# pixeli99/SVD_Xtend

Hardware: AMD Instinct MI355X
Metric: train-step samples/sec (14-frame 512x320 fp16 SVD UNet) (higher is better)
Workload: dtype fp16; 1 GPU; SVD UNet train step, 14 frames 512x320, batch 1/GPU, 1524623082 params (397620480 trainable: temporal_transformer_block*), fwd + EDM loss + bwd + grad all-reduce + AdamW; global_batch=1, grad_accum=1, parallelism=dp1, grad_allreduce=none, ranks_seen=1, allreduce_bytes=1590482176, exec=hipgraph, gemm_tuning_sweeps=0, gemm_variant=4

## Files before the change

include/svdx.h:

```cpp
#ifndef SVDX_H
#define SVDX_H
#include <stddef.h>
#include <stdint.h>

#ifdef __cplusplus
extern "C" {
#endif

#define SVDX_F16 0
#define SVDX_BF16 1

#define SVDX_OUT_ACT 0
#define SVDX_OUT_F32 1
#define SVDX_OUT_F32_ATOMIC 2
#define SVDX_OUT_F32_ADD 4
#define SVDX_OUT_F32_SLAB 3

#define SVDX_EPI_NONE 0
#define SVDX_EPI_GEGLU_FWD 1
#define SVDX_EPI_GEGLU_BWD 2

#define SVDX_GATHER_PLAIN 0
#define SVDX_GATHER_CONV3X3 1
#define SVDX_GATHER_CONV3X3_DGRAD2 2
#define SVDX_GATHER_TEMPORAL3 3
#define SVDX_GATHER_CONV3X3_PAD0 4

typedef struct svdx_gather {
    int mode;
    int n_img;
    int hi, wi;
    int ho, wo;
    int cin;
    int stride;
    int ups;
    int t, hw;
    int lda;
} svdx_gather;

#define SVDX_VERSION 614
int         svdx_version(void);
int         svdx_last_error(char* buf, size_t n);
int         svdx_device_ok(void);

int svdx_gemm(const void* A, const void* B, void* C, int M, int N, int K, int lda, int ldb, int ldc,
              const float* bias, const float* rowvec, int rv_ld, int rv_rows_per_group, int rv_mod,
              const void* res, int ldres, const svdx_gather* gather, const void* zero_page,
              int out_mode, float alpha, int split_k, int variant, int epilogue, const void* aux_in, void* aux_out, int aux_dim,
              int dtype, void* stream);
int svdx_gemm_tile(int variant, int M, int N, int split_k, int epilogue, int aux_dim, int* geom);

int svdx_gemm_gn(const void* A, const void* B, void* C, int M, int N, int K, int lda, int ldb, int ldc,
                 const float* bias, const float* rowvec, int rv_ld, int rv_rows_per_group, int rv_mod,
                 const void* res, int ldres, const svdx_gather* gather, const void* zero_page,
                 float alpha, int variant, float* gn_stats, int gn_rows, int gn_cg, int dtype, void* stream);

int svdx_gemm_dual(const void* A, const void* B, void* C, int M, int N, int K, int lda, int ldb, int ldc,
                   const float* bias, const float* rowvec, int rv_ld, int rv_rows_per_group, int rv_mod,
                   const void* res, int ldres, const svdx_gather* gather, const void* zero_page,
                   int out_mode, float alpha, int variant, const void* A2, const void* B2, int K2, int lda2, int ldb2,
                   int a2_seg_n, int dtype, void* stream);

#define SVDX_TN_FLAT 64
int svdx_gemm_tn(const void* A, const void* B, float* C, int R, int N, int K, int lda, int ldb, int ldc,
                 float* a_colsum, const void* zero_page, int out_mode, int split_k, int stages, float* found_inf, int dtype, void* stream);

int svdx_gemm_tn_gather(const void* A, const void* X, float* C, int R, int N, int lda, int ldc, const svdx_gather* gather,
                        float* a_colsum, int out_mode, int split_k, int stages, float* found_inf, int dtype, void* stream);

int svdx_conv_wgrad_finalize(const float* acc, int nsplit, int64_t slab_stride, int ld_acc, float* w_grad, int cout, int cin, int cin_p,
                             int taps, float alpha, int store, const float* colsum_slabs, int colsum_ld, float* b_grad, float* found_inf,
                             void* stream);

// ... 85 lines not shown
                     const float* lse, const float* D, void* dq, int nb, int heads, int S,
                     int ld, int ld_o, int ld_d, float scale, int dtype, void* stream);

int svdx_tattn_fwd(const void* q, const void* k, const void* v, void* o, int B, int T, int HW, int heads,
                   int ld, int ld_o, float scale, int dtype, void* stream);
int svdx_tattn_bwd(const void* q, const void* k, const void* v, const void* d_o, void* dq, void* dk, void* dv,
                   int B, int T, int HW, int heads, int ld, int ld_o, int ld_d, float scale, int dtype, void* stream);

int svdx_geglu_fwd(const void* pre, void* out, int M, int F, int dtype, void* stream);
int svdx_geglu_bwd(const void* dout, const void* pre, void* dpre, int M, int F, int dtype, void* stream);
int svdx_add(const void* a, const void* b, void* out, int64_t n, int dtype, void* stream);
int svdx_blend(const void* a, const void* b, const float* mix_factor, void* out, int64_t n, int dtype, void* stream);
int svdx_blend_bwd(const void* dy, const float* mix_factor, void* da, void* db, int64_t n, int dtype, void* stream);
int svdx_add_rowvec(const void* x, const float* vec, void* out, int rows, int C, int rv_ld,
                    int rows_per_group, int mod, int dtype, void* stream);
#define SVDX_COLSUM_SLAB 512
int svdx_colsum(const void* x, float* out, int rows, int C, int ldx, int n_groups, int rows_per_group, int mod,
                int accumulate, float* scratch, int dtype, void* stream);
int svdx_transpose(const void* in, int ld_in, void* out, int ld_out, int rows, int cols, int dtype, void* stream);
int svdx_concat2(const void* a, int Ca, const void* b, int Cb, void* out, int rows, int dtype, void* stream);
int svdx_split2(const void* in, void* a, int Ca, void* b, int Cb, int rows, int dtype, void* stream);
int svdx_sum2x2(const void* in, void* out, int n_img, int h, int w, int C, int dtype, void* stream);
int svdx_cast_from_f32(const float* in, void* out, int64_t n, int dtype, void* stream);
int svdx_cast_transpose_from_f32(const float* in, void* out, int R, int Ccols, int dtype, void* stream);
int svdx_nchw_to_rows(const float* in, void* out, int n_img, int C, int H, int W, int ld, float mul, int dtype, void* stream);
int svdx_rows_to_nchw(const void* in, float* out, int n_img, int C, int H, int W, int ld, int dtype, void* stream);
int svdx_zero(void* p, size_t bytes, void* stream);

int svdx_tsa_pixels_per_band(int T, int HW);
int svdx_tsa_fwd(const void* x, const float* gamma, const float* beta, float eps, const void* wqkv, const void* wo, const float* bo,
                 const float* cvec, int rv_ld, int rv_rows_per_group, int rv_mod, void* n1, float* stats, void* qkv, void* o, void* h1,
                 int B, int T, int HW, int C, int heads, float scale, int dtype, void* stream);

int svdx_patch_rows(const float* in, void* out, int n_img, int C, int H, int W, int kh, int kw, int stride, int pad, int ho, int wo,
                    int ldk, float mul, int dtype, void* stream);
int svdx_softmax_rows(const void* in, void* out, int rows, int cols, int cols_out, int64_t ld_in, int64_t ld_out, float scale,
                      int dtype, void* stream);
int svdx_act_rows(const void* in, void* out, int64_t n, int act, int dtype, void* stream);
int svdx_blur_axis(const float* in, float* out, int planes, int H, int W, const float* taps, int ntaps, int axis, void* stream);
int svdx_bicubic_affine(const float* in, float* out, int n_img, int C, int H, int W, int ho, int wo, const float* scale,
                        const float* shift, void* stream);
int svdx_attn_small_fwd(const void* qkv, void* out, int n_img, int S, int heads, int d, int dp, int64_t ld, int64_t ld_o, float scale,
                        int dtype, void* stream);
int svdx_zero_spans(float* base, const int* spans, int n_spans, void* stream);
int svdx_stamp(uint64_t* slot, void* stream);
int svdx_wall_clock_khz(void);

int     svdx_plan_begin(void);
int     svdx_plan_end(void** plan);
int64_t svdx_plan_launches(const void* plan);
int64_t svdx_plan_bytes(const void* plan);
int     svdx_plan_replay(const void* plan, void* stream);
int     svdx_plan_free(void* plan);

#define SVDX_MAX_PEERS 16
int svdx_allreduce_grads(float* const* peers, int world, int rank, int64_t n, int phase, void* stream);

#define SVDX_EDM_LOSS_SCRATCH 1024
int svdx_edm_loss(const void* pred, int ld, const float* noisy, const float* target, const float* sigma,
                  float* loss, void* dpred, int B, int T, int C, int HW, const float* opt_state, float* scratch,
                  int dtype, void* stream);

#define SVDX_OPT_STATE_FLOATS 16
#define SVDX_SCHED_CONSTANT 0
#define SVDX_SCHED_CONSTANT_WITH_WARMUP 1
#define SVDX_SCHED_LINEAR 2
// ... 35 lines not shown
```

svd_xtend_amd/build.py:

```python
from __future__ import annotations

import os
import subprocess
import sys
from concurrent.futures import ThreadPoolExecutor

HERE = os.path.dirname(os.path.abspath(__file__))
CSRC = os.path.join(HERE, "csrc")
SOURCES = ["common.cpp", "gemm_nt.hip", "gemm_tn.hip", "gemm_small.hip", "norm.hip", "elementwise.hip", "attention.hip", "tattn.hip", "optim.hip", "encoders.hip", "tsa.hip", "latent.hip", "conv_wgrad.hip"]
FLAGS = ["--offload-arch=gfx950", "-O3", "-std=c++17", "-fPIC", "-Wno-unused-value"]
LIB = os.path.join(CSRC, "libsvdx.so")


def _stale(out: str, deps) -> bool:
    if not os.path.exists(out):
        return True
    t = os.path.getmtime(out)
    return any(os.path.getmtime(d) > t for d in deps)


def build(force: bool = False, verbose: bool = False) -> str:
    hipcc = os.environ.get("HIPCC", "/opt/rocm/bin/hipcc")
    hdrs = sorted(os.path.join(CSRC, f) for f in os.listdir(CSRC) if f.endswith(".h")) + [os.path.join(HERE, "..", "include", "svdx.h")]
    objs = []

    def compile_one(src):
        s = os.path.join(CSRC, src)
        o = os.path.join(CSRC, os.path.splitext(src)[0] + ".o")
        if force or _stale(o, [s] + hdrs):
            cmd = [hipcc] + FLAGS + (["-x", "hip"] if src.endswith(".cpp") else []) + ["-c", s, "-o", o]
            if verbose:
                print(" ".join(cmd), flush=True)
            r = subprocess.run(cmd, capture_output=True, text=True)
            if r.returncode != 0:
                raise RuntimeError(f"hipcc failed on {src}:\n{r.stderr}")
        return o

    with ThreadPoolExecutor(max_workers=6) as ex:
        objs = list(ex.map(compile_one, SOURCES))
    if force or _stale(LIB, objs):
        cmd = [hipcc, "--offload-arch=gfx950", "-shared", "-fPIC", "-o", LIB] + objs
        r = subprocess.run(cmd, capture_output=True, text=True)
# ... 8 lines not shown
```

svd_xtend_amd/kernels.py:

```python
from __future__ import annotations

import ctypes
import os
from dataclasses import dataclass
from typing import Optional

import torch

_HERE = os.path.dirname(os.path.abspath(__file__))
LIB_PATH = os.environ.get("SVDX_LIB") or os.path.join(_HERE, "csrc", "libsvdx.so")

F16, BF16 = 0, 1
OUT_ACT, OUT_F32, OUT_F32_ATOMIC, OUT_F32_SLAB, OUT_F32_ADD = 0, 1, 2, 3, 4
EPI_NONE, EPI_GEGLU_FWD, EPI_GEGLU_BWD = 0, 1, 2
LN_PARTIAL_ROWS = 2048
GN_REPLICAS = 8
GN_STAT_FLOATS = 4
GATHER_PLAIN, GATHER_CONV3X3, GATHER_CONV3X3_DGRAD2, GATHER_TEMPORAL3, GATHER_CONV3X3_PAD0 = 0, 1, 2, 3, 4
ABI_VERSION = 614
OPT_STATE_FLOATS = 16
SCHED_KINDS = {"constant": 0, "constant_with_warmup": 1, "linear": 2, "cosine": 3, "cosine_with_restarts": 4, "polynomial": 5, "piecewise_constant": 6}
SCHED_MAX_RULES = 8
OPT_STATE_ALLOC = 40


class SvdxError(RuntimeError):
    pass


class _LinJobC(ctypes.Structure):
    _fields_ = [("X", ctypes.c_void_p), ("W", ctypes.c_void_p), ("bias", ctypes.c_void_p), ("Y", ctypes.c_void_p),
                ("N", ctypes.c_int), ("K", ctypes.c_int), ("ldw", ctypes.c_int), ("flags", ctypes.c_int)]


class _OuterJobC(ctypes.Structure):
    _fields_ = [("dY", ctypes.c_void_p), ("X", ctypes.c_void_p), ("dW", ctypes.c_void_p),
                ("N", ctypes.c_int), ("K", ctypes.c_int), ("scale", ctypes.c_float), ("reserved", ctypes.c_int)]


class _GradFinJobC(ctypes.Structure):
    _fields_ = [("acc", ctypes.c_void_p), ("dst", ctypes.c_void_p), ("colsum_slabs", ctypes.c_void_p), ("colsum_out", ctypes.c_void_p),
                ("slab_stride", ctypes.c_int64), ("count", ctypes.c_int64), ("nsplit", ctypes.c_int), ("colsum_n", ctypes.c_int),
                ("store", ctypes.c_int), ("reserved", ctypes.c_int), ("found_inf", ctypes.c_void_p)]


class _LnRedJobC(ctypes.Structure):
    _fields_ = [("partial", ctypes.c_void_p), ("dgamma", ctypes.c_void_p), ("dbeta", ctypes.c_void_p),
                ("nblk", ctypes.c_int), ("C", ctypes.c_int)]


class _GatherC(ctypes.Structure):
    _fields_ = [(n, ctypes.c_int) for n in
# ... 21 lines not shown


_SIGS = {
    "svdx_gemm": "ppp" "iiiiii" "p" "piii" "pi" "pp" "ifii" "ippi" "ip",
    "svdx_gemm_dual": "ppp" "iiiiii" "p" "piii" "pi" "pp" "ifi" "pp" "iiii" "ip",
    "svdx_gemm_gn": "ppp" "iiiiii" "p" "piii" "pi" "pp" "fi" "pii" "ip",
    "svdx_gemm_tn": "ppp" "iiiiii" "pp" "iii" "p" "ip",
    "svdx_gemm_tn_gather": "ppp" "iiii" "pp" "iii" "p" "ip",
    "svdx_conv_wgrad_finalize": "pil" "ip" "iiii" "fi" "pi" "pp" "p",
    "svdx_conv_pack": "pf" "pp" "iiiii" "i" "pp" "ip",
    "svdx_gemm_finalize": "pil" "pi" "iii" "pp" "iii" "pi" "ppi" "ip",
    "svdx_gemm_finalize_gn": "pil" "p" "iii" "pp" "iii" "pi" "pii" "ip",
    "svdx_small_linear": "pppp" "iiii" "iii" "ip",
    "svdx_outer_acc": "ppp" "iii" "f" "p",
    "svdx_small_linear_batch": "p" "iii" "ip",
    "svdx_outer_acc_batch": "p" "ii" "p",
    "svdx_ln_param_reduce_batch": "p" "i" "p",
    "svdx_grad_finalize_batch": "p" "i" "p",
    "svdx_timestep_embed": "pp" "ii" "p",
    "svdx_gn_stats": "pp" "iiii" "i" "ip",
    "svdx_gn_apply": "ppppp" "iiii" "fi" "ip",
    "svdx_gn_bwd_stats": "pppppp" "iiii" "fi" "i" "ip",
    "svdx_gn_bwd_apply": "pppppppp" "iiii" "fi" "ip",
    "svdx_gn_bwd_stats_affine": "ppppppppp" "iiii" "fi" "ii" "ip",
    "svdx_ln_fwd": "ppppp" "ii" "f" "ip",
    "svdx_ln_bwd": "pppppp" "f" "pppp" "iii" "ip",
    "svdx_attn_fwd": "ppppp" "iiiii" "f" "ip",
    "svdx_attn_bwd_prep": "ppp" "iii" "i" "ip",
    "svdx_attn_bwd_dkv": "pppppppp" "iiiiii" "f" "ip",
    "svdx_attn_bwd_dq": "ppppppp" "iiiiii" "f" "ip",
    "svdx_tattn_fwd": "pppp" "iiii" "ii" "f" "ip",
    "svdx_tattn_bwd": "ppppppp" "iiii" "iii" "f" "ip",
    "svdx_tsa_fwd": "ppp" "f" "ppp" "piii" "ppppp" "iiiii" "f" "ip",
    "svdx_geglu_fwd": "pp" "ii" "ip",
    "svdx_geglu_bwd": "ppp" "ii" "ip",
    "svdx_add": "ppp" "l" "ip",
    "svdx_blend": "pppp" "l" "ip",
    "svdx_blend_bwd": "pppp" "l" "ip",
    "svdx_add_rowvec": "ppp" "iiiii" "ip",
    "svdx_colsum": "pp" "iiiiiii" "p" "ip",
    "svdx_transpose": "pi" "pi" "ii" "ip",
    "svdx_concat2": "pi" "pi" "p" "i" "ip",
    "svdx_split2": "p" "pi" "pi" "i" "ip",
    "svdx_sum2x2": "pp" "iiii" "ip",
    "svdx_cast_from_f32": "pp" "l" "ip",
    "svdx_cast_transpose_from_f32": "pp" "ii" "ip",
    "svdx_nchw_to_rows": "pp" "iiiii" "f" "ip",
    "svdx_rows_to_nchw": "pp" "iiiii" "ip",
    "svdx_zero": "pzp",
    "svdx_patch_rows": "pp" "iiiiiiiiii" "i" "f" "ip",
    "svdx_softmax_rows": "pp" "iii" "ll" "f" "ip",
    "svdx_act_rows": "pp" "l" "i" "ip",
    "svdx_blur_axis": "pp" "iii" "p" "ii" "p",
    "svdx_bicubic_affine": "pp" "iiiiii" "pp" "p",
    "svdx_attn_small_fwd": "pp" "iiiii" "ll" "f" "ip",
    "svdx_stamp": "pp",
    "svdx_zero_spans": "pp" "ip",
    "svdx_edm_loss": "pi" "ppppp" "iiii" "pp" "ip",
    "svdx_check_finite": "plpp",
    "svdx_check_finite_spans": "pp" "i" "pp",
    "svdx_optim_prep": "p" "ffff" "ii" "p",
    "svdx_adamw": "pppp" "l" "dddddd" "pp" "iip",
    "svdx_adamw_tiled": "ppppp" "i" "dddddd" "ppp" "iip",
    "svdx_ema_lerp": "pp" "l" "f" "p",
    "svdx_latent_batch": "pp" "i" "p" "pp" "pp" "ppp" "f" "ppp" "iii" "p",
    "svdx_grad_sumsq_spans": "pp" "i" "pp",
    "svdx_grad_clip_coef": "pp" "ii" "dd" "pp" "ip",
    "svdx_allreduce_grads": "p" "ii" "l" "i" "p",
    "svdx_plan_begin": "",
    "svdx_plan_end": "p",
    "svdx_plan_replay": "pp",
    "svdx_plan_free": "p",
}
_CT = {"p": ctypes.c_void_p, "i": ctypes.c_int, "f": ctypes.c_float, "d": ctypes.c_double, "l": ctypes.c_int64, "z": ctypes.c_size_t}

EXPORTED_SYMBOLS = tuple(_SIGS) + ("svdx_wall_clock_khz", "svdx_version", "svdx_last_error", "svdx_device_ok", "svdx_tsa_pixels_per_band", "svdx_ln_bwd_blocks", "svdx_gn_bwd_blocks", "svdx_gemm_tile",
                                    "svdx_plan_launches", "svdx_plan_bytes")
PARAMS_F32, PARAMS_BF16_REFERENCE = 0, 1
TN_FLAT = 64
MAX_PEERS = 16
CLIP_SPAN_FLOATS = 65536
CLIP_MAX_TENSORS = 8192
BATCH_MAX_JOBS = 48
TSA_MAX_C, TSA_MAX_T, TSA_BAND_ROWS = 320, 16, 144


COLSUM_SLAB = 512
EDM_LOSS_SCRATCH = 1024


def colsum_slabs(rows: int, rpg: int, mod: int) -> int:
    maxcnt = -(-rows // mod) if mod else min(rpg, rows)
    return -(-maxcnt // COLSUM_SLAB)


def ln_bwd_blocks(rows: int, C: int) -> int:
    cc = C // 8
    lanes = 16 if cc <= 48 else (32 if cc <= 96 else 64)
    per, cap = 1, min(512, LN_PARTIAL_ROWS)
    return max(1, min(-(-rows // (per * (256 // lanes))), cap))


GN_AFFINE_MIN_SLAB, GN_AFFINE_SMALL_SLAB, GN_AFFINE_MIN_BLOCKS = 16, 4, 256


def gn_bwd_blocks(n_s: int, rows: int, C: int, G: int = 32) -> int:
    rpi = 1 if C // 8 >= 256 else 256 // (C // 8)
    slab = 64
    while slab > 2 * rpi and slab > GN_AFFINE_MIN_SLAB and n_s * -(-rows // slab) < 512:
        slab >>= 1
    while slab > 2 * rpi and slab > GN_AFFINE_SMALL_SLAB and n_s * -(-rows // slab) < GN_AFFINE_MIN_BLOCKS:
        slab >>= 1
    return n_s * -(-rows // slab)


def tsa_pixels_per_band(T: int, HW: int) -> int:
    if T <= 0 or T > TSA_MAX_T or HW <= 0:
# ... 225 lines not shown
                   _f32(dgamma), _f32(dbeta), _f32(scratch), rows, C, int(defer_reduce), _dt(x), self._stream())

    def ln_param_reduce_batch(self, jobs):
        arr = (_LnRedJobC * len(jobs))(*[_LnRedJobC(_f32(pt), _f32(dg), _f32(db), nblk, C) for pt, dg, db, nblk, C in jobs])
        self._call("svdx_ln_param_reduce_batch", ctypes.cast(arr, ctypes.c_void_p), len(jobs), self._stream())

    def attn_fwd(self, q, k, v, o, lse, nb, heads, S, ld, ld_o, scale):
        self._call("svdx_attn_fwd", _p(q), _p(k), _p(v), _p(o), _f32(lse), nb, heads, S, ld, ld_o,
                   float(scale), _dt(q), self._stream())

    def attn_bwd_prep(self, o, d_o, D, nb, heads, S, ld_o):
        self._call("svdx_attn_bwd_prep", _p(o), _p(d_o), _f32(D), nb, heads, S, ld_o, _dt(o), self._stream())

    def attn_bwd_dkv(self, q, k, v, d_o, lse, D, dk, dv, nb, heads, S, ld, ld_o, ld_d, scale):
        self._call("svdx_attn_bwd_dkv", _p(q), _p(k), _p(v), _p(d_o), _f32(lse), _f32(D),
                   _p(dk), _p(dv), nb, heads, S, ld, ld_o, ld_d, float(scale), _dt(q), self._stream())

    def attn_bwd_dq(self, q, k, v, d_o, lse, D, dq, nb, heads, S, ld, ld_o, ld_d, scale):
        self._call("svdx_attn_bwd_dq", _p(q), _p(k), _p(v), _p(d_o), _f32(lse), _f32(D), _p(dq),
                   nb, heads, S, ld, ld_o, ld_d, float(scale), _dt(q), self._stream())

    def tattn_fwd(self, q, k, v, o, B, T, HW, heads, ld, ld_o, scale):
        self._call("svdx_tattn_fwd", _p(q), _p(k), _p(v), _p(o), B, T, HW, heads, ld, ld_o, float(scale),
                   _dt(q), self._stream())

    def tattn_bwd(self, q, k, v, d_o, dq, dk, dv, B, T, HW, heads, ld, ld_o, ld_d, scale):
        self._call("svdx_tattn_bwd", _p(q), _p(k), _p(v), _p(d_o), _p(dq), _p(dk), _p(dv), B, T, HW, heads,
                   ld, ld_o, ld_d, float(scale), _dt(q), self._stream())

    def tsa_fwd(self, x, gamma, beta, eps, wqkv, wo, bo, cvec, rv_ld, rv_rpg, rv_mod, n1, stats, qkv, o, h1, B, T, HW, C, heads, scale):
        self._call("svdx_tsa_fwd", _p(x), _f32(gamma), _f32(beta), float(eps), _p(wqkv), _p(wo), _f32(bo), _f32(cvec), rv_ld, rv_rpg,
                   rv_mod, _p(n1), _f32(stats), _p(qkv), _p(o), _p(h1), B, T, HW, C, heads, float(scale), _dt(x), self._stream())

    def geglu_fwd(self, pre, out, M, F):
        self._call("svdx_geglu_fwd", _p(pre), _p(out), M, F, _dt(pre), self._stream())

    def geglu_bwd(self, dout, pre, dpre, M, F):
        self._call("svdx_geglu_bwd", _p(dout), _p(pre), _p(dpre), M, F, _dt(pre), self._stream())

    def add(self, a, b, out, n):
        self._call("svdx_add", _p(a), _p(b), _p(out), n, _dt(a), self._stream())

    def blend(self, a, b, mix, out, n):
        self._call("svdx_blend", _p(a), _p(b), _f32(mix), _p(out), n, _dt(a), self._stream())

    def blend_bwd(self, dy, mix, da, db, n):
        self._call("svdx_blend_bwd", _p(dy), _f32(mix), _p(da), _p(db), n, _dt(dy), self._stream())

    def add_rowvec(self, x, vec, out, rows, C, rv_ld, rpg, mod):
        self._call("svdx_add_rowvec", _p(x), _f32(vec), _p(out), rows, C, rv_ld, rpg, mod, _dt(x), self._stream())

    def colsum(self, x, out, rows, C, ldx, n_groups, rpg, mod, accumulate=0, scratch=None):
        if scratch is not None:
            assert scratch.numel() >= colsum_slabs(rows, rpg, mod) * n_groups * C
        self._call("svdx_colsum", _p(x), _f32(out), rows, C, ldx, n_groups, rpg, mod, int(accumulate), _f32(scratch), _dt(x),
                   self._stream())

    def transpose(self, inp, ld_in, out, ld_out, rows, cols):
        self._call("svdx_transpose", _p(inp), ld_in, _p(out), ld_out, rows, cols, _dt(inp), self._stream())

    def concat2(self, a, Ca, b, Cb, out, rows):
        self._call("svdx_concat2", _p(a), Ca, _p(b), Cb, _p(out), rows, _dt(a), self._stream())

    def split2(self, inp, a, Ca, b, Cb, rows):
        self._call("svdx_split2", _p(inp), _p(a), Ca, _p(b), Cb, rows, _dt(inp), self._stream())

# ... 134 lines not shown
```

svd_xtend_amd/ops.py:

```python
from __future__ import annotations

import contextlib
import functools
import os
from dataclasses import dataclass
from types import SimpleNamespace
from typing import List, NamedTuple, Optional, Sequence

import torch
import torch.nn as nn

from . import kernels as K

GN_GROUPS = 32


def rup(x: int, m: int) -> int:
    return (x + m - 1) // m * m


def _layout_order(names: List[str]) -> List[int]:
    first, keys = {}, []
    for i, n in enumerate(names):
        if ".lora_A." in n or ".lora_B." in n:
# ... 2 lines not shown
        else:
            keys.append((i, 0, i))
    return sorted(range(len(names)), key=lambda i: keys[i])


def flatten_trainables(model: "nn.Module", align: int = 64):
    named = [(n, p) for n, p in model.named_parameters() if p.requires_grad]
    params = [p for _, p in named]
    dev = params[0].device if params else next(model.parameters()).device
    offs, off = [0] * len(params), 0
    for i in _layout_order([n for n, _ in named]):
        offs[i] = off
        off = rup(off + params[i].numel(), align)
    p_flat = torch.zeros(off + align, dtype=torch.float32, device=dev)
    g_flat = torch.zeros(off + align, dtype=torch.float32, device=dev)
    for p, o in zip(params, offs):
        n = p.numel()
        p_flat[o:o + n].copy_(p.data.reshape(-1))
        p.data = p_flat[o:o + n].view(p.shape)
        p.grad = g_flat[o:o + n].view(p.shape)
    return params, offs, off, p_flat, g_flat


class Runtime:

    def __init__(self, dtype: torch.dtype, device: torch.device):
        self.dt = dtype
        self.dev = device
        self.k = K.backend()
        self.gemm_variant = 4
        self.split_k = True
        self.fuse_geglu = True
        self.fuse_tsa = True
        self.fuse_dual = True
        self.lora_stack_da = True
        self.tuner = None
        self.wt16_flat = None
        self.wt_pos = 0
        self.wt_map = {}
        self.adam_writes_wt = False
        self.grad_overwrite = False
        self.grads_fresh = False
        self.write_once = set()
        self.arenas = [None, None]
        self.arena_cap = 1 << 20
        self.arena_cur, self.arena_pos = None, 0
        self.batch_small = True
        self.dvec_from_dw = True
        self._q_nn, self._q_outer, self._q_ln, self._q_M, self._q_outer_dst = [], [], [], None, set()
        self._q_fin, self._q_fin_dst, self._q_fin_bytes = [], set(), 0
        self.defer_grad_finalize = True
        self.found_inf = None
        self.fold_finite = True
        self.unchecked_grads = False
        self.fin_queue_budget = 768 << 20
        self.fuse_gn_stats = True
        self.p_flat = None
        self.w16_flat = None

    on_region = None

    @contextlib.contextmanager
    def region(self, name: str, **info):
        cb = self.on_region
        if cb is None:
            yield
# ... 987 lines not shown
```

svd_xtend_amd/train.py:

```python
from __future__ import annotations

import os
import warnings
from typing import Dict, List, Optional

import torch
import torch.distributed as dist

from . import kernels as K
from .ops import flatten_trainables
from .unet import UNetSpatioTemporalConditionModel

ALIGN = 64


DEFAULT_TRAINABLE = "temporal_transformer_block"


def select_trainable(model: torch.nn.Module, which="temporal_transformer_block") -> List[str]:
    rules = [which] if isinstance(which, str) else list(which)
    if not rules or not all(isinstance(r, str) and r for r in rules):
        raise ValueError(f"trainable={which!r}: a non-empty string or a sequence of them")
    has_lora = any(".lora_" in name for name, _ in model.named_parameters())
    conv = set()
# ... 156 lines not shown
        self.n_flat = off
        self.n_total = off + ALIGN
        self.m_flat = torch.zeros(self.n_total, dtype=torch.float32, device=dev)
        self.v_flat = torch.zeros(self.n_total, dtype=torch.float32, device=dev)
        self.loss_slot = self.g_flat[off:off + 1]
        self.dynamic = dtype == torch.float16
        st = [0.0] * K.OPT_STATE_ALLOC
        st[1], st[4], st[5], st[6], st[8] = (init_scale if self.dynamic else 1.0), 1.0, 1.0, 1.0, 1.0
        self.opt_state = torch.tensor(st, dtype=torch.float32, device=dev)
        self.clip_out = torch.zeros(2, dtype=torch.float32, device=dev) if self.max_grad_norm is not None else None
        self.grad_norm = self.clip_out[0] if self.clip_out is not None else None
        self.clip_coef = self.clip_out[1] if self.clip_out is not None else None
        self.micro = 0
        self.schedule = dict(name="constant", num_warmup_steps=0, num_training_steps=0, num_cycles=0.0, power=1.0, lr_end=1e-7,
                             steps_per_step=1)
        src = (dist.get_global_rank(process_group, 0) if process_group is not None else 0) if self.world > 1 else 0
        if self.world > 1:
            for t in list(model.parameters()) + list(model.buffers()):
                if not t.requires_grad:
                    dist.broadcast(t.data, src=src, group=process_group)
        if self.param_mode == K.PARAMS_BF16_REFERENCE:
            self.p_flat.copy_(self.p_flat.to(torch.bfloat16).to(torch.float32))
        self._build_runtime()
        if self.world > 1:
            dist.broadcast(self.p_flat, src=src, group=process_group)
            self.weights_changed()

    def _build_runtime(self) -> None:
        model, dtype, dev = self.model, self.dtype, self.dev
        old = getattr(self, "rt", None)
        model.prepare(dtype)
        self.rt = model.rt
        if old is not None:
            for knob in ("tuner", "gemm_variant", "split_k", "fuse_geglu", "fuse_dual", "fuse_tsa"):
                setattr(self.rt, knob, getattr(old, knob))
        tiled = bool(self.params)
        self.adam_tiles = build_adam_tiles(self.params, self.offsets, self.rt.wt_map, dev) if tiled else None
        self.rt.adam_writes_wt = self.adam_tiles is not None
        spans, pos = [], 0
        for off, p in sorted(zip(self.offsets, self.params), key=lambda t: t[0]):
            if id(p) in self.rt.write_once:
                if off > pos:
                    spans.append((pos, off))
                pos = off + p.numel()
        if self.n_total > pos:
            spans.append((pos, self.n_total))
        chunks = []
        for lo, hi in spans:
            lo4, hi4 = lo // 4 * 4, -(-hi // 4) * 4
            for c in range(lo4, hi4, 1 << 16):
                chunks.append((c, min(1 << 16, hi4 - c)))
        self.zero_spans = torch.tensor(chunks, dtype=torch.int32, device=dev).contiguous() if self.rt.write_once else None
        fin = [(c, min(n, self.n_flat - c)) for c, n in chunks if c < self.n_flat]
        self.finite_spans = torch.tensor(fin, dtype=torch.int32, device=dev).contiguous() if (self.rt.write_once and fin) else None
        self.rt.found_inf = self.opt_state[3:4] if (self.world == 1 and self.zero_spans is not None) else None
        self.clip_spans = self.clip_partial = None
        self.n_clip_tensors = 0
        if self.max_grad_norm is not None and self.params:
            rows = []
            for i, (p, off) in enumerate(zip(self.params, self.offsets)):
                assert off % 4 == 0 and off + p.numel() <= self.n_flat
                rows += [(off + c, min(K.CLIP_SPAN_FLOATS, p.numel() - c), i) for c in range(0, p.numel(), K.CLIP_SPAN_FLOATS)]
            if len(self.params) > K.CLIP_MAX_TENSORS:
                raise ValueError(f"gradient clipping: {len(self.params)} trainable tensors, the kernel takes {K.CLIP_MAX_TENSORS}")
            self.clip_spans = torch.tensor(rows, dtype=torch.int32).contiguous().to(dev)
            self.clip_partial = torch.zeros(len(rows), dtype=torch.float64, device=dev)
            self.n_clip_tensors = len(self.params)
# ... 374 lines not shown
```

svd_xtend_amd/unet.py:

```python
from __future__ import annotations

from types import SimpleNamespace
from typing import List, Optional, Tuple

import torch
import torch.nn as nn

from . import kernels as K
from .lora import LoraLinear, base_linear, inject
from .ops import _ones as ops_ones
from .ops import (ConvOp, GroupNormOp, LayerNormOp, LinearOp, LoraOp, Runtime, SmallLinearOp, SmallLoraOp, choose_geglu_variant, geglu_candidates, choose_split, flatten_trainables, tuned_call,
                  rup)
from .pretrained import CONFIG_NAME, WEIGHTS_NAME, FrozenConfig, PretrainedMixin

HEAD_DIM = 64


class Geom:

    def __init__(self, B: int, T: int, h: int, w: int):
        self.B, self.T, self.h, self.w = B, T, h, w
        self.N = B * T
        self.HW = h * w
        self.M = self.N * self.HW
# ... 24 lines not shown
        self.mix_factor = nn.Parameter(torch.tensor([0.5], dtype=torch.float32))


class _GEGLU(nn.Module):
    def __init__(self, dim, inner):
        super().__init__()
        self.proj = nn.Linear(dim, inner * 2)


class _FeedForward(nn.Module):

    def __init__(self, dim, dim_out=None):
        super().__init__()
        self.dim, self.inner = dim, dim * 4
        self.net = nn.ModuleList([_GEGLU(dim, self.inner), nn.Dropout(0.0), nn.Linear(self.inner, dim_out or dim)])

    def build(self):
        self.p1 = LinearOp([self.net[0].proj.weight], [self.net[0].proj.bias])
        self.p2 = LinearOp([self.net[2].weight], [self.net[2].bias])

    def pack(self, rt):
        self.p1.pack(rt)
        self.p2.pack(rt)

    def refresh(self, rt):
        for op in (self.p1, self.p2):
            if op.trainable:
                op.refresh(rt)

    def _fusable(self, rt, M):
        F = self.inner
        return (rt.gemm_variant == 4 and rt.fuse_geglu and F % 128 == 0 and choose_split(rt, M, 2 * F, self.dim, 2 * F) == 1
                and choose_split(rt, M, F, self.p2.N, 2 * F) == 1)

    def fwd(self, rt, x, M, res):
        F = self.inner
        g = rt.empty(M, F)
        if self._fusable(rt, M):
            pre = rt.empty(M, 2 * F)
            tuned_call(rt, ("geglu_fwd", M, F, self.dim), lambda: geglu_candidates(M, 2 * F, self.dim),
                       lambda: choose_geglu_variant(M, 2 * F, self.dim),
                       lambda v: rt.k.gemm(x, self.p1.w, pre, M, 2 * F, self.dim, self.dim, self.dim, 2 * F, bias=self.p1.b, variant=v,
                                           epilogue=K.EPI_GEGLU_FWD, aux_out=g, aux_dim=F))
        else:
            pre = self.p1.fwd(rt, x, M)
            rt.k.geglu_fwd(pre, g, M, F)
        y = self.p2.fwd(rt, g, M, res=res)
        return y, pre, g

    def fwd_ln(self, rt, ln, x, M, res, need_n: bool):
        n, st = ln.fwd(rt, x, M)
        y, pre, g = self.fwd(rt, n, M, res)
        return y, pre, g, n, st

    def bwd(self, rt, dy, x_saved, pre, g, M):
        k = rt.k
        F = self.inner
        dpre = rt.empty(M, 2 * F)
        if self._fusable(rt, M):
            tuned_call(rt, ("geglu_bwd", M, F, self.p2.N), lambda: geglu_candidates(M, F, self.p2.N, fwd=False),
                       lambda: choose_geglu_variant(M, F, self.p2.N, fwd=False),
                       lambda v: k.gemm(dy, self.p2.wt, dpre, M, F, self.p2.N, self.p2.N, self.p2.N, 2 * F, variant=v,
                                        epilogue=K.EPI_GEGLU_BWD, aux_in=pre, aux_dim=F))
        else:
            dg = self.p2.bwd_dx(rt, dy, M)
            k.geglu_bwd(dg, pre, dpre, M, F)
            del dg
        if self.p2.trainable:
            self.p2.bwd_dw(rt, dy, g, M)
        dx = self.p1.bwd_dx(rt, dpre, M)
        if self.p1.trainable:
            self.p1.bwd_dw(rt, dpre, x_saved, M)
        return dx


class HipAttnProcessor:

    def __repr__(self):
        return "HipAttnProcessor()"


class _Attention(nn.Module):
    def __init__(self, dim, heads, cross_dim=None):
        super().__init__()
        self.processor = HipAttnProcessor()
        inner = heads * HEAD_DIM
        kv = cross_dim if cross_dim is not None else dim
        self.heads, self.dim, self.cross = heads, dim, cross_dim is not None
        self.to_q = nn.Linear(dim, inner, bias=False)
        self.to_k = nn.Linear(kv, inner, bias=False)
# ... 1203 lines not shown
```

Measured before the change: 20.99 samples/s.

## Fuse FFN backward GEGLU-dgrad chain into one banded kernel for C=320

Adds a dedicated HIP kernel that, per band of rows, computes dg = dy·W2ᵀ into LDS, applies the GEGLU backward in registers, and immediately multiplies the resulting dpre chunk by W1ᵀ to accumulate dx. The aim is to avoid writing and re-reading the full M×2F dpre tensor, and to cut launches, when p1 is frozen. The path only applies when dim=320, F=1280, and either p1 is not trainable or the dpre-store option is enabled. It trades general tuned GEMMs for a hand-scheduled kernel whose MFMA efficiency at this size is uncertain.

```diff
diff --git a/include/svdx.h b/include/svdx.h
--- a/include/svdx.h
+++ b/include/svdx.h
@@ -38,7 +38,7 @@
     int lda;
 } svdx_gather;
 
-#define SVDX_VERSION 614
+#define SVDX_VERSION 615
 int         svdx_version(void);
 int         svdx_last_error(char* buf, size_t n);
 int         svdx_device_ok(void);
@@ -190,6 +190,9 @@
                  const float* cvec, int rv_ld, int rv_rows_per_group, int rv_mod, void* n1, float* stats, void* qkv, void* o, void* h1,
                  int B, int T, int HW, int C, int heads, float scale, int dtype, void* stream);
 
+int svdx_ffn_bwd(const void* dy, const void* pre, const void* w2t, const void* w1t, void* dpre_out, void* dx, int M, int C, int F,
+                 int dtype, void* stream);
+
 int svdx_patch_rows(const float* in, void* out, int n_img, int C, int H, int W, int kh, int kw, int stride, int pad, int ho, int wo,
                     int ldk, float mul, int dtype, void* stream);
 int svdx_softmax_rows(const void* in, void* out, int rows, int cols, int cols_out, int64_t ld_in, int64_t ld_out, float scale,
diff --git a/svd_xtend_amd/build.py b/svd_xtend_amd/build.py
--- a/svd_xtend_amd/build.py
+++ b/svd_xtend_amd/build.py
@@ -7,7 +7,7 @@
 
 HERE = os.path.dirname(os.path.abspath(__file__))
 CSRC = os.path.join(HERE, "csrc")
-SOURCES = ["common.cpp", "gemm_nt.hip", "gemm_tn.hip", "gemm_small.hip", "norm.hip", "elementwise.hip", "attention.hip", "tattn.hip", "optim.hip", "encoders.hip", "tsa.hip", "latent.hip", "conv_wgrad.hip"]
+SOURCES = ["common.cpp", "gemm_nt.hip", "gemm_tn.hip", "gemm_small.hip", "norm.hip", "elementwise.hip", "attention.hip", "tattn.hip", "optim.hip", "encoders.hip", "tsa.hip", "ffn.hip", "latent.hip", "conv_wgrad.hip"]
 FLAGS = ["--offload-arch=gfx950", "-O3", "-std=c++17", "-fPIC", "-Wno-unused-value"]
 LIB = os.path.join(CSRC, "libsvdx.so")
 
diff --git a/svd_xtend_amd/csrc/ffn.hip b/svd_xtend_amd/csrc/ffn.hip
--- /dev/null
+++ b/svd_xtend_amd/csrc/ffn.hip
@@ -0,0 +1,247 @@
+#include "common.h"
+#include "band.h"
+
+namespace {
+
+constexpr int FFN_C = 320;
+constexpr int FFN_KB = FFN_C / 64;
+constexpr int FFN_WAVES = 4;
+constexpr int FFN_NT = 64 * FFN_WAVES;
+constexpr int FFN_FC = 16 * FFN_WAVES;
+constexpr int FFN_KS1 = FFN_C / 32;
+constexpr int FFN_NJ = FFN_C / 16 / FFN_WAVES;
+constexpr int FFN_IMG = FFN_KB * TSA_RP * 128;
+constexpr int FFN_DH = TSA_RP * FFN_FC * 2;
+constexpr int FFN_DP = TSA_RP * FFN_FC * 4;
+constexpr int FFN_LDS = FFN_IMG + FFN_DH + FFN_DP;
+constexpr int FFN_UNITS = TSA_RP * (FFN_FC / 8);
+constexpr int FFN_NIT = (FFN_UNITS + FFN_NT - 1) / FFN_NT;
+static_assert(FFN_NIT >= 4, "the gate pass carries the four request groups of S3's B fragments, one per unit");
+
+struct FfnParams {
+    const void* dy; const void* pre; const void* w2t; const void* w1t; void* dpre; void* dx;
+    int M, F;
+};
+
+template <typename T>
+__global__ __launch_bounds__(FFN_NT) void ffn_bwd_kernel(FfnParams p) {
+#if defined(__HIP_DEVICE_COMPILE__)
+    extern __shared__ __attribute__((aligned(16))) char smem[];
+    typedef typename TT<T>::v8 v8;
+    const int tid = threadIdx.x, lane = tid & 63, wave = __builtin_amdgcn_readfirstlane(tid >> 6), fr = lane & 15, fg = lane >> 4;
+    const int F = p.F, F2 = 2 * F;
+    char* IMG = smem;
+    char* DH = smem + FFN_IMG;
+    char* DP = DH + FFN_DH;
+    const int row0 = blockIdx.x * TSA_RP;
+    const int R = min(TSA_RP, p.M - row0);
+    auto grow = [&](int lr) __attribute__((always_inline)) { return row0 + lr; };
+    __amdgpu_buffer_rsrc_t rsP = __builtin_amdgcn_make_buffer_rsrc(const_cast<void*>(p.pre), 0, p.M * F2 * 2, 0x00020000);
+    __amdgpu_buffer_rsrc_t rsD = __builtin_amdgcn_make_buffer_rsrc(p.dpre ? p.dpre : const_cast<void*>(p.pre), 0, p.dpre ? p.M * F2 * 2 : 0, 0x00020000);
+    __amdgpu_buffer_rsrc_t rsW2 = __builtin_amdgcn_make_buffer_rsrc(const_cast<void*>(p.w2t), 0, F * FFN_C * 2, 0x00020000);
+    __amdgpu_buffer_rsrc_t rsW1 = __builtin_amdgcn_make_buffer_rsrc(const_cast<void*>(p.w1t), 0, FFN_C * F2 * 2, 0x00020000);
+    __amdgpu_buffer_rsrc_t rsX = __builtin_amdgcn_make_buffer_rsrc(p.dx, 0, p.M * FFN_C * 2, 0x00020000);
+
+    int g_off[FFN_NIT], g_lds[FFN_NIT], g_dp[FFN_NIT];
+#pragma unroll
+    for (int it = 0; it < FFN_NIT; ++it) {
+        const int u = min(it * FFN_NT + tid, FFN_UNITS - 1), row = u >> 3, seg = u & 7;
+        g_off[it] = row < R ? (grow(row) * F2 + seg * 8) * 2 : TSA_OOB;
+        g_lds[it] = row * 128 + ((seg ^ (row & 7)) * 16);
+        g_dp[it] = row * 256 + ((seg ^ (row & 15)) * 16);
+    }
+    auto unit_on = [&](int it) __attribute__((always_inline)) { return it * FFN_NT + wave * 64 < FFN_UNITS; };
+    tsa_u4 pa[FFN_NIT], pg[FFN_NIT];
+    auto load_pre = [&](int f0) __attribute__((always_inline)) {
+#pragma unroll
+        for (int it = 0; it < FFN_NIT; ++it) {
+            const int off = unit_on(it) ? g_off[it] : TSA_OOB;
+            pa[it] = __builtin_amdgcn_raw_buffer_load_b128(rsP, off + f0 * 2, 0, 2);
+            pg[it] = __builtin_amdgcn_raw_buffer_load_b128(rsP, off + (F + f0) * 2, 0, 2);
+        }
+    };
+    const int b1_off = ((wave * 16 + fr) * FFN_C + fg * 8) * 2;
+    tsa_u4 b1[FFN_KS1];
+    auto load_b1 = [&](int f0) __attribute__((always_inline)) {
+#pragma unroll
+        for (int s = 0; s < FFN_KS1; ++s) b1[s] = __builtin_amdgcn_raw_buffer_load_b128(rsW2, b1_off + (f0 * FFN_C + s * 32) * 2, 0, 0);
+    };
+    const int b2_off = ((wave * 16 + fr) * F2 + fg * 8) * 2;
+    tsa_u4 b2[2][2][FFN_NJ];
+    auto load_b2 = [&](int f0, int q) __attribute__((always_inline)) {
+#pragma unroll
+        for (int j = 0; j < FFN_NJ; ++j)
+            b2[q >> 1][q & 1][j] = __builtin_amdgcn_raw_buffer_load_b128(rsW1, b2_off + (j * FFN_WAVES * 16 * F2 + (q >> 1) * F + f0 + (q & 1) * 32) * 2, 0, 0);
+    };
+    auto lds_barrier = [&]() __attribute__((always_inline)) {
+        asm volatile("s_waitcnt lgkmcnt(0)" ::: "memory");
+        __builtin_amdgcn_s_barrier();
+        asm volatile("" ::: "memory");
+    };
+
+    load_b1(0);
+    load_pre(0);
+    band_load<FFN_KB>(IMG, p.dy, p.M * FFN_C * 2, R, grow, tid);
+    band_load<FFN_KB>(IMG, p.dy, p.M * FFN_C * 2, R, grow, tid + FFN_NT);
+
+    f32x4 acc2[FFN_NJ][TSA_MB];
+#pragma unroll
+    for (int j = 0; j < FFN_NJ; ++j)
+#pragma unroll
+        for (int i = 0; i < TSA_MB; ++i) acc2[j][i] = f32x4{0.f, 0.f, 0.f, 0.f};
+    const char* A1 = IMG + fr * 128;
+    const char* A2 = DP + fr * 256;
+    const int sw = fr & 7;
+
+#ifdef FFN_STAMPS
+    unsigned long long st[8] = {0, 0, 0, 0, 0, 0, 0, 0}, t_ = __builtin_readcyclecounter(), t0_ = t_;
+#define FFN_ST(i) do { const unsigned long long n_ = __builtin_readcyclecounter(); st[i] += n_ - t_; t_ = n_; } while (0)
+#else
+#define FFN_ST(i) do { } while (0)
+#endif
+    for (int f0 = 0; f0 < F; f0 += FFN_FC) {
+        FFN_ST(5);
+        {
+            f32x4 acc1[TSA_MB];
+#pragma unroll
+            for (int i = 0; i < TSA_MB; ++i) acc1[i] = f32x4{0.f, 0.f, 0.f, 0.f};
+            v8 a[2][TSA_MB];
+            auto read_a = [&](int s) __attribute__((always_inline)) {
+                const char* As = A1 + (s >> 1) * (TSA_RP * 128) + ((((s & 1) * 4 + fg) ^ sw) * 16);
+#pragma unroll
+                for (int i = 0; i < TSA_MB; ++i) a[s & 1][i] = *reinterpret_cast<const v8*>(As + i * (16 * 128));
+            };
+            read_a(0);
+#pragma unroll
+            for (int s = 0; s < FFN_KS1; ++s) {
+                if (s + 1 < FFN_KS1) read_a(s + 1);
+                const v8 b = __builtin_bit_cast(v8, b1[s]);
+#pragma unroll
+                for (int i = 0; i < TSA_MB; ++i) acc1[i] = TT<T>::mfma(b, a[s & 1][i], acc1[i]);
+            }
+            __builtin_amdgcn_sched_group_barrier(0x100, TSA_MB, 0);
+#pragma unroll
+            for (int k = 0; k < (FFN_KS1 - 1) * TSA_MB; ++k) {
+                __builtin_amdgcn_sched_group_barrier(0x008, 1, 0);
+                __builtin_amdgcn_sched_group_barrier(0x100, 1, 0);
+            }
+            __builtin_amdgcn_sched_group_barrier(0x008, TSA_MB, 0);
+#pragma unroll
+            for (int i = 0; i < TSA_MB; ++i) {
+                const int row = i * 16 + fr;
+                Vec4<T> o;
+#pragma unroll
+                for (int e = 0; e < 4; ++e) o.v[e] = from_f<T>(acc1[i][e]);
+                *reinterpret_cast<Vec4<T>*>(DH + row * 128 + (((wave * 2 + (fg >> 1)) ^ sw) * 16) + (fg & 1) * 8) = o;
+            }
+        }
+        FFN_ST(0);
+        lds_barrier();
+        FFN_ST(1);
+#pragma unroll
+        for (int it = 0; it < FFN_NIT; ++it) {
+            if (it < 4) load_b2(f0, it);
+            if (unit_on(it)) {
+                const Vec8<T> d8 = *reinterpret_cast<const Vec8<T>*>(DH + g_lds[it]);
+                const Vec8<T> a8 = __builtin_bit_cast(Vec8<T>, pa[it]), g8 = __builtin_bit_cast(Vec8<T>, pg[it]);
+                Vec8<T> da, dg;
+#pragma unroll
+                for (int e = 0; e < 8; ++e) {
+                    const float d = to_f<T>(d8.v[e]), gv = to_f<T>(g8.v[e]);
+                    const GeluParts gp = gelu_parts(gv);
+                    da.v[e] = from_f<T>(d * gv * gp.cdf);
+                    dg.v[e] = from_f<T>(d * to_f<T>(a8.v[e]) * (gp.cdf + gp.pdf_x));
+                }
+                *reinterpret_cast<Vec8<T>*>(DP + g_dp[it]) = da;
+                *reinterpret_cast<Vec8<T>*>(DP + (g_dp[it] ^ 128)) = dg;
+                if (p.dpre) {
+                    tsa_store16(__builtin_bit_cast(tsa_u4, da), rsD, g_off[it] + f0 * 2, 0);
+                    tsa_store16(__builtin_bit_cast(tsa_u4, dg), rsD, g_off[it] + (F + f0) * 2, 0);
+                }
+            }
+        }
+        FFN_ST(2);
+        lds_barrier();
+        FFN_ST(3);
+        {
+            const int fn = f0 + FFN_FC < F ? f0 + FFN_FC : 0;
+            load_pre(fn);
+            load_b1(fn);
+        }
+        {
+            v8 a[2][TSA_MB];
+            auto read_a = [&](int q) __attribute__((always_inline)) {
+                const char* As = A2 + (((q * 4 + fg) ^ fr) * 16);
+#pragma unroll
+                for (int i = 0; i < TSA_MB; ++i) a[q & 1][i] = *reinterpret_cast<const v8*>(As + i * (16 * 256));
+            };
+            read_a(0);
+#pragma unroll
+            for (int q = 0; q < 4; ++q) {
+                if (q + 1 < 4) read_a(q + 1);
+#pragma unroll
+                for (int i = 0; i < TSA_MB; ++i)
+#pragma unroll
+                    for (int j = 0; j < FFN_NJ; ++j)
+                        acc2[j][i] = TT<T>::mfma(__builtin_bit_cast(v8, b2[q >> 1][q & 1][j]), a[q & 1][i], acc2[j][i]);
+            }
+            __builtin_amdgcn_sched_group_barrier(0x100, TSA_MB, 0);
+#pragma unroll
+            for (int k = 0; k < 3 * TSA_MB; ++k) {
+                __builtin_amdgcn_sched_group_barrier(0x008, FFN_NJ, 0);
+                __builtin_amdgcn_sched_group_barrier(0x100, 1, 0);
+                if (k < 2 * FFN_NIT + FFN_KS1) __builtin_amdgcn_sched_group_barrier(0x020, 1, 0);
+            }
+            __builtin_amdgcn_sched_group_barrier(0x008, FFN_NJ * TSA_MB, 0);
+        }
+    }
+
+    FFN_ST(4);
+#pragma unroll
+    for (int j = 0; j < FFN_NJ; ++j)
+#pragma unroll
+        for (int i = 0; i < TSA_MB; ++i) {
+            Vec4<T> o;
+#pragma unroll
+            for (int e = 0; e < 4; ++e) o.v[e] = from_f<T>(acc2[j][i][e]);
+            *reinterpret_cast<Vec4<T>*>(IMG + (i * 16 + fr) * (FFN_C * 2) + ((wave + FFN_WAVES * j) * 16 + fg * 4) * 2) = o;
+        }
+    lds_barrier();
+    for (int u = tid; u < TSA_RP * (FFN_C / 8); u += FFN_NT) {
+        const int row = u / (FFN_C / 8), ch = u - row * (FFN_C / 8);
+        const tsa_u4 v = *reinterpret_cast<const tsa_u4*>(IMG + u * 16);
+        tsa_store16(v, rsX, row < R ? (grow(row) * FFN_C + ch * 8) * 2 : TSA_OOB, 0);
+    }
+#ifdef FFN_STAMPS
+    asm volatile("s_waitcnt vmcnt(0)" ::: "memory");
+    __syncthreads();
+    st[6] = __builtin_readcyclecounter() - t0_;
+    if (lane == 0 && R == TSA_RP) for (int i = 0; i < 8; ++i) reinterpret_cast<unsigned long long*>(p.dx)[(size_t)row0 * 80 + wave * 8 + i] = st[i];
+#endif
+#endif
+}
+
+}
+
+extern "C" int svdx_ffn_bwd(const void* dy, const void* pre, const void* w2t, const void* w1t, void* dpre_out, void* dx, int M, int C, int F,
+                            int dtype, void* stream) {
+    SVDX_CHECK_ARG(dy && pre && w2t && w1t && dx, "svdx_ffn_bwd: null argument");
+    SVDX_CHECK_ARG(M >= 1 && C == FFN_C && F >= FFN_FC && F % FFN_FC == 0, "svdx_ffn_bwd: needs C = %d and F a multiple of %d (got C=%d F=%d)",
+                   FFN_C, FFN_FC, C, F);
+    SVDX_CHECK_ARG((((uintptr_t)dy | (uintptr_t)pre | (uintptr_t)w2t | (uintptr_t)w1t | (uintptr_t)dpre_out | (uintptr_t)dx) & 15) == 0,
+                   "svdx_ffn_bwd: operands must be 16-byte aligned");
+    SVDX_CHECK_ARG((long)M * 2 * F * 2 < (1L << 31), "svdx_ffn_bwd: activation too large for 32-bit buffer offsets");
+    FfnParams p;
+    p.dy = dy; p.pre = pre; p.w2t = w2t; p.w1t = w1t; p.dpre = dpre_out; p.dx = dx; p.M = M; p.F = F;
+    const int blocks = cdiv(M, TSA_RP);
+    DISPATCH_DTYPE(dtype, {
+        static bool attr_set = false;
+        if (!attr_set) {
+            (void)hipFuncSetAttribute(reinterpret_cast<const void*>(&ffn_bwd_kernel<T>), hipFuncAttributeMaxDynamicSharedMemorySize, FFN_LDS);
+            attr_set = true;
+        }
+        hipLaunchKernelGGL((ffn_bwd_kernel<T>), dim3(blocks), dim3(FFN_NT), FFN_LDS, (hipStream_t)stream, p);
+    });
+    SVDX_LAUNCH_CHECK("svdx_ffn_bwd");
+    return 0;
+}
diff --git a/svd_xtend_amd/kernels.py b/svd_xtend_amd/kernels.py
--- a/svd_xtend_amd/kernels.py
+++ b/svd_xtend_amd/kernels.py
@@ -17,7 +17,7 @@
 GN_REPLICAS = 8
 GN_STAT_FLOATS = 4
 GATHER_PLAIN, GATHER_CONV3X3, GATHER_CONV3X3_DGRAD2, GATHER_TEMPORAL3, GATHER_CONV3X3_PAD0 = 0, 1, 2, 3, 4
-ABI_VERSION = 614
+ABI_VERSION = 615
 OPT_STATE_FLOATS = 16
 SCHED_KINDS = {"constant": 0, "constant_with_warmup": 1, "linear": 2, "cosine": 3, "cosine_with_restarts": 4, "polynomial": 5, "piecewise_constant": 6}
 SCHED_MAX_RULES = 8
@@ -105,6 +105,7 @@
     "svdx_tattn_fwd": "pppp" "iiii" "ii" "f" "ip",
     "svdx_tattn_bwd": "ppppppp" "iiii" "iii" "f" "ip",
     "svdx_tsa_fwd": "ppp" "f" "ppp" "piii" "ppppp" "iiiii" "f" "ip",
+    "svdx_ffn_bwd": "pppppp" "iii" "ip",
     "svdx_geglu_fwd": "pp" "ii" "ip",
     "svdx_geglu_bwd": "ppp" "ii" "ip",
     "svdx_add": "ppp" "l" "ip",
@@ -156,6 +157,7 @@
 CLIP_MAX_TENSORS = 8192
 BATCH_MAX_JOBS = 48
 TSA_MAX_C, TSA_MAX_T, TSA_BAND_ROWS = 320, 16, 144
+FFN_BWD_C, FFN_BAND_ROWS = 320, 144
 
 
 COLSUM_SLAB = 512
@@ -447,6 +449,9 @@
         self._call("svdx_tsa_fwd", _p(x), _f32(gamma), _f32(beta), float(eps), _p(wqkv), _p(wo), _f32(bo), _f32(cvec), rv_ld, rv_rpg,
                    rv_mod, _p(n1), _f32(stats), _p(qkv), _p(o), _p(h1), B, T, HW, C, heads, float(scale), _dt(x), self._stream())
 
+    def ffn_bwd(self, dy, pre, w2t, w1t, dpre_out, dx, M, C, F):
+        self._call("svdx_ffn_bwd", _p(dy), _p(pre), _p(w2t), _p(w1t), _p(dpre_out), _p(dx), M, C, F, _dt(dy), self._stream())
+
     def geglu_fwd(self, pre, out, M, F):
         self._call("svdx_geglu_fwd", _p(pre), _p(out), M, F, _dt(pre), self._stream())
 
diff --git a/svd_xtend_amd/ops.py b/svd_xtend_amd/ops.py
--- a/svd_xtend_amd/ops.py
+++ b/svd_xtend_amd/ops.py
@@ -58,6 +58,8 @@
         self.split_k = True
         self.fuse_geglu = True
         self.fuse_tsa = True
+        self.fuse_ffn_bwd = True
+        self.fuse_ffn_bwd_dpre = False
         self.fuse_dual = True
         self.lora_stack_da = True
         self.tuner = None
diff --git a/svd_xtend_amd/train.py b/svd_xtend_amd/train.py
--- a/svd_xtend_amd/train.py
+++ b/svd_xtend_amd/train.py
@@ -212,7 +212,7 @@
         model.prepare(dtype)
         self.rt = model.rt
         if old is not None:
-            for knob in ("tuner", "gemm_variant", "split_k", "fuse_geglu", "fuse_dual", "fuse_tsa"):
+            for knob in ("tuner", "gemm_variant", "split_k", "fuse_geglu", "fuse_dual", "fuse_tsa", "fuse_ffn_bwd", "fuse_ffn_bwd_dpre"):
                 setattr(self.rt, knob, getattr(old, knob))
         tiled = bool(self.params)
         self.adam_tiles = build_adam_tiles(self.params, self.offsets, self.rt.wt_map, dev) if tiled else None
diff --git a/svd_xtend_amd/unet.py b/svd_xtend_amd/unet.py
--- a/svd_xtend_amd/unet.py
+++ b/svd_xtend_amd/unet.py
@@ -80,6 +80,11 @@
         F = self.inner
         return (rt.gemm_variant == 4 and rt.fuse_geglu and F % 128 == 0 and choose_split(rt, M, 2 * F, self.dim, 2 * F) == 1
                 and choose_split(rt, M, F, self.p2.N, 2 * F) == 1)
+
+    def _ffn_bwd_fusable(self, rt, M):
+        F = self.inner
+        return (self._fusable(rt, M) and rt.fuse_ffn_bwd and hasattr(rt.k, "ffn_bwd") and self.dim == K.FFN_BWD_C and F == 4 * K.FFN_BWD_C
+                and self.p2.N == K.FFN_BWD_C and M * 2 * F * 2 < 2 ** 31 and (rt.fuse_ffn_bwd_dpre or not self.p1.trainable))
 
     def fwd(self, rt, x, M, res):
         F = self.inner
@@ -104,6 +109,15 @@
     def bwd(self, rt, dy, x_saved, pre, g, M):
         k = rt.k
         F = self.inner
+        if self._ffn_bwd_fusable(rt, M):
+            dpre = rt.empty(M, 2 * F) if self.p1.trainable else None
+            dx = rt.empty(M, self.dim)
+            k.ffn_bwd(dy, pre, self.p2.wt, self.p1.wt, dpre, dx, M, self.dim, F)
+            if self.p2.trainable:
+                self.p2.bwd_dw(rt, dy, g, M)
+            if self.p1.trainable:
+                self.p1.bwd_dw(rt, dpre, x_saved, M)
+            return dx
         dpre = rt.empty(M, 2 * F)
         if self._fusable(rt, M):
             tuned_call(rt, ("geglu_bwd", M, F, self.p2.N), lambda: geglu_candidates(M, F, self.p2.N, fwd=False),
```

Result: no change. 21.01 samples/s (median of 6 runs) (+0.1%).
